# lightalchemist/nonlocal-image-edit

Hardware: AMD Instinct MI355X
Metric: megapixels/sec end-to-end enhance (4K img, m=200, K=50); device-resident input and output (host->host per SURVEY 8d: host_to_host.value) (higher is better)
Workload: dtype f64; 1 GPU; cfg4: 4096x4096 synthetic luminance, 20x10 samples (p=200), K=50, T=10, L=4 layers; device-resident: the luminance plane is in HBM when the timed region starts and the 4 layer planes are left in HBM (no PCIe inside `value`); parallelism=single GPU, formulation=phi_free_tables, storage=fp64 tables, histograms, reductions and MFMA; fp32 output planes

## Files before the change

### include/nle.h

```cpp
#ifndef NLE_H
#define NLE_H

#include <stddef.h>

#ifdef __cplusplus
extern "C" {
#endif

#define NLE_OK 0
#define NLE_ERR_INVALID 1
#define NLE_ERR_HIP 2
#define NLE_ERR_NUMERIC 3
#define NLE_ERR_COMM 4

#define NLE_EPS 1e-10

typedef struct nle_ctx nle_ctx;
typedef struct nle_filter nle_filter;

int nle_ctx_create(int device, void* stream, nle_ctx** out);
void nle_ctx_destroy(nle_ctx* ctx);
const char* nle_last_error(const nle_ctx* ctx);
int nle_ctx_synchronize(nle_ctx* ctx);
int nle_ctx_trim(nle_ctx* ctx);
// ... 87 lines not shown
                         double hy, int form, double thresh, float* d_r, double* h_summary);
int nle_ts_gemm64(nle_ctx* ctx, const double* d_A, long long M, int lda, int kd, const double* h_B, int nc, double* d_C);
int nle_sinkhorn_scalings64(nle_ctx* ctx, const double* d_phi, long long M, int ld, int r, const double* h_eigvals,
                            int max_iter, double* h_u_c, double* h_u_r);
int nle_gram64(nle_ctx* ctx, const double* d_phi, long long M, int ld, int r, const double* h_u, double* h_G);
int nle_row_scalings64(nle_ctx* ctx, const double* d_phi, long long M, int ld, int r, const double* h_u, double* d_out);
int nle_sample_pass(nle_ctx* ctx, const float* d_lum, int H, int W, int n_row_samples, int n_col_samples, double hx, double hy,
                    int row0, int row1, int recip, const double* h_w, double* d_y, double* h_z);
int nle_sample_gram(nle_ctx* ctx, const float* d_lum, int H, int W, int n_row_samples, int n_col_samples, double hx, double hy,
                    int row0, int row1, const double* d_c, double* h_G);
int nle_sample_project(nle_ctx* ctx, const float* d_lum, int H, int W, int n_row_samples, int n_col_samples, double hx,
                       double hy, int row0, int row1, const double* h_D, int K, const double* d_c, float* d_V, int ldv);
int nle_sample_update(nle_ctx* ctx, int p, int r, int chol, int recip, const double* h_X1, const double* h_X2,
                      const double* h_lam, const double* h_z, int zrows, int zld, const double* h_sA, double* h_v, double* h_u,
                      double* h_sA_next, double* h_w_next);
long long nle_table_workspace(int n_sel_rows, int n_sel_cols, int nrows, int gram);
int nle_table_levels(nle_ctx* ctx, const float* d_x, long long n, int* h_bad, unsigned* h_mask);
int nle_table_build(nle_ctx* ctx, const float* d_lum, int H, int W, int n_row_samples, int n_col_samples, int row0, int row1,
                    double hx, double hy, const double* d_er, const double* d_ecT, const double* d_Ep, const double* d_cvec,
                    double* d_er_out, double* d_ecT_out, double* d_Ep_out, int* h_info);
int nle_table_pass(nle_ctx* ctx, const float* d_lum, int H, int W, int n_row_samples, int n_col_samples, int row0, int row1,
                   double hx, double hy, const double* d_er, const double* d_ecT, const double* d_Ep, const double* d_cvec,
                   int mode, const double* d_w, const float* d_xvec, double* d_y, double* d_ws, long long ws_elems, double* d_z);
int nle_table_expand(nle_ctx* ctx, const float* d_lum, int H, int W, int n_row_samples, int n_col_samples, int row0, int row1,
                     double hx, double hy, const double* d_er, const double* d_ecT, const double* d_Ep, const double* d_cvec,
                     const double* d_wl, int ldw, int nl, int round8, double* d_gws, float* d_out, long long ostride);
int nle_table_gram(nle_ctx* ctx, const float* d_lum, int H, int W, int n_row_samples, int n_col_samples, int row0, int row1,
                   double hx, double hy, const double* d_er, const double* d_ecT, const double* d_Ep, const double* d_cvec,
                   double* d_ws, long long ws_elems, double* d_Gk, int* h_split);
int nle_table_apply_small(nle_ctx* ctx, int p, int K, int ldk, int L, int ldw, const double* d_m, const double* d_D,
// ... 132 lines not shown
```

### nonlocal-image-edit_amd/__init__.py

```python
from __future__ import annotations

import ctypes as C
import os

import numpy as np

_HERE = os.path.dirname(os.path.abspath(__file__))
LIB_PATH = os.path.join(_HERE, "lib", "libnle_hip.so")

from . import _abi
from ._abi import (ALLREDUCE_FN, NLE_ERR_COMM, NLE_ERR_HIP, NLE_ERR_INVALID, NLE_ERR_NUMERIC, NLE_OK)

EPS = 1e-10
KERNEL_COUNT = _abi.NLE_KERNEL_COUNT
_P = C.c_void_p
_SIGNATURES = _abi.SIGNATURES
EXPORTED_SYMBOLS = tuple(_SIGNATURES)
MODE_AUTO, MODE_MATERIALISED, MODE_PHI_FREE, MODE_PHI_FREE_EXP, MODE_MATERIALISED_F64, MODE_STREAMED_F64 = (
    _abi.NLE_MODE_AUTO, _abi.NLE_MODE_MATERIALISED, _abi.NLE_MODE_PHI_FREE, _abi.NLE_MODE_PHI_FREE_EXP,
    _abi.NLE_MODE_MATERIALISED_F64, _abi.NLE_MODE_STREAMED_F64)
MODE_EXACT_F64 = _abi.NLE_MODE_EXACT_F64
EXACT_MAX_PIXELS = _abi.NLE_EXACT_MAX_PIXELS
SAMPLER_GRID, SAMPLER_FARTHEST = _abi.NLE_SAMPLER_GRID, _abi.NLE_SAMPLER_FARTHEST
SAMPLER_RESIDUAL = _abi.NLE_SAMPLER_RESIDUAL
# ... 638 lines not shown
        X1c, X2r = np.asfortranarray(X), np.ascontiguousarray(np.asarray(X2, dtype=np.float64))
        n2, r = X.shape
        p = n2 // 2
        lam = np.ascontiguousarray(lam, dtype=np.float64)
        z = np.ascontiguousarray(np.atleast_2d(z), dtype=np.float64)
        sA = None if sA is None else np.ascontiguousarray(sA, dtype=np.float64)
        if n2 != 2 * p or X2r.shape != (n2, r) or lam.size != r or z.shape[1] < p or (sA is not None and sA.size != p):
            raise NLEError(NLE_ERR_INVALID, "sample_update: X1, X2 (2p x r), lam (r), z (zrows x zld >= p), sA (p)")
        v, u, sn, wn = np.zeros(n2), np.zeros(r), np.zeros(p), np.zeros(p)
        self._sync_in()
        _check(lib().nle_sample_update(self._h, p, r, int(bool(chol)), int(sA is not None), _np_ptr(X1c), _np_ptr(X2r),
                                       _np_ptr(lam), _np_ptr(z), z.shape[0], z.shape[1], _np_ptr(sA) if sA is not None else None,
                                       _np_ptr(v), _np_ptr(u), _np_ptr(sn), _np_ptr(wn)), self._h)
        return v, u, sn, wn

    def _dev64(self, a, what, n=None):
        if a is None:
            return None
        torch = _torch()
        t = torch.as_tensor(a, dtype=torch.float64, device=f"cuda:{self.device}").contiguous()
        if n is not None and t.numel() != n:
            raise NLEError(NLE_ERR_INVALID, f"{what}: need {n} doubles, got {t.numel()}")
        return t

    def _table_view(self, lum, nr, nc, rows, tables, hx, hy, c, who):
        t, H, W = self._plane(lum)
        row0, row1 = rows if rows is not None else (0, H)
        g = sample_grid(H, W, nr, nc)
        nR, nC, nrows = g["n_sel_rows"], g["n_sel_cols"], max(row1 - row0, 0)
        keep = [t]
# ... 606 lines not shown
```

### nonlocal-image-edit_amd/_abi.py

```python
import ctypes as C

_P = C.c_void_p

NLE_OK = 0
NLE_ERR_INVALID = 1
NLE_ERR_HIP = 2
NLE_ERR_NUMERIC = 3
NLE_ERR_COMM = 4
NLE_MODE_AUTO = 0
NLE_MODE_MATERIALISED = 1
NLE_MODE_PHI_FREE = 2
NLE_MODE_PHI_FREE_EXP = 3
NLE_MODE_MATERIALISED_F64 = 4
NLE_MODE_STREAMED_F64 = 5
NLE_MODE_EXACT_F64 = 6
NLE_EXACT_MAX_PIXELS = 1048576
NLE_PATCH_RADIUS_MAX = 7
NLE_CHROMA_PATCH_RADIUS_MAX = 3
NLE_SAMPLER_GRID = 0
NLE_SAMPLER_FARTHEST = 1
NLE_SAMPLER_RESIDUAL = 3
NLE_RCCL_UNIQUE_ID_BYTES = 128
NLE_RESID_AUTO = 0
NLE_RESID_ROWS = 1
# ... 73 lines not shown
    "nle_nystrom": (C.c_int, [_P, _P, C.c_int, C.c_int, C.c_int, C.c_int, C.c_double, C.c_double, _P, _P, _P]),
    "nle_ts_gemm": (C.c_int, [_P, _P, C.c_longlong, C.c_int, C.c_int, _P, C.c_int, _P]),
    "nle_sinkhorn_scalings": (C.c_int, [_P, _P, C.c_longlong, C.c_int, C.c_int, _P, C.c_int, _P, _P]),
    "nle_gram": (C.c_int, [_P, _P, C.c_longlong, C.c_int, C.c_int, _P, _P]),
    "nle_row_scalings": (C.c_int, [_P, _P, C.c_longlong, C.c_int, C.c_int, _P, _P]),
    "nle_compute_kernel64": (C.c_int, [_P, _P, C.c_int, C.c_int, C.c_int, C.c_int, C.c_double, C.c_double, _P, _P]),
    "nle_nystrom_residual": (C.c_int, [_P, _P, C.c_int, C.c_int, C.c_int, C.c_int, C.c_double, C.c_double, C.c_int, C.c_double, _P, _P]),
    "nle_ts_gemm64": (C.c_int, [_P, _P, C.c_longlong, C.c_int, C.c_int, _P, C.c_int, _P]),
    "nle_sinkhorn_scalings64": (C.c_int, [_P, _P, C.c_longlong, C.c_int, C.c_int, _P, C.c_int, _P, _P]),
    "nle_gram64": (C.c_int, [_P, _P, C.c_longlong, C.c_int, C.c_int, _P, _P]),
    "nle_row_scalings64": (C.c_int, [_P, _P, C.c_longlong, C.c_int, C.c_int, _P, _P]),
    "nle_sample_pass": (C.c_int, [_P, _P, C.c_int, C.c_int, C.c_int, C.c_int, C.c_double, C.c_double, C.c_int, C.c_int, C.c_int, _P, _P, _P]),
    "nle_sample_gram": (C.c_int, [_P, _P, C.c_int, C.c_int, C.c_int, C.c_int, C.c_double, C.c_double, C.c_int, C.c_int, _P, _P]),
    "nle_sample_project": (C.c_int, [_P, _P, C.c_int, C.c_int, C.c_int, C.c_int, C.c_double, C.c_double, C.c_int, C.c_int, _P, C.c_int, _P, _P, C.c_int]),
    "nle_sample_update": (C.c_int, [_P, C.c_int, C.c_int, C.c_int, C.c_int, _P, _P, _P, _P, C.c_int, C.c_int, _P, _P, _P, _P, _P]),
    "nle_table_workspace": (C.c_longlong, [C.c_int, C.c_int, C.c_int, C.c_int]),
    "nle_table_levels": (C.c_int, [_P, _P, C.c_longlong, _P, _P]),
    "nle_table_build": (C.c_int, [_P, _P, C.c_int, C.c_int, C.c_int, C.c_int, C.c_int, C.c_int, C.c_double, C.c_double, _P, _P, _P, _P, _P, _P, _P, _P]),
    "nle_table_pass": (C.c_int, [_P, _P, C.c_int, C.c_int, C.c_int, C.c_int, C.c_int, C.c_int, C.c_double, C.c_double, _P, _P, _P, _P, C.c_int, _P, _P, _P, _P, C.c_longlong, _P]),
    "nle_table_expand": (C.c_int, [_P, _P, C.c_int, C.c_int, C.c_int, C.c_int, C.c_int, C.c_int, C.c_double, C.c_double, _P, _P, _P, _P, _P, C.c_int, C.c_int, C.c_int, _P, _P, C.c_longlong]),
    "nle_table_gram": (C.c_int, [_P, _P, C.c_int, C.c_int, C.c_int, C.c_int, C.c_int, C.c_int, C.c_double, C.c_double, _P, _P, _P, _P, _P, C.c_longlong, _P, _P]),
    "nle_table_apply_small": (C.c_int, [_P, C.c_int, C.c_int, C.c_int, C.c_int, C.c_int, _P, _P, _P, _P, _P, _P, _P, _P, _P, _P, _P]),
    "nle_table_scatter": (C.c_int, [_P, C.c_int, C.c_int, _P, _P, _P, C.c_longlong, C.c_int]),
    "nle_gemm64s": (C.c_int, [_P, C.c_int, C.c_int, C.c_int, _P, C.c_longlong, C.c_longlong, _P, C.c_longlong, C.c_longlong, _P, C.c_longlong, C.c_longlong, _P, _P, _P, _P, C.c_longlong, C.c_longlong]),
    "nle_gemm64s_window": (C.c_int, []),
    "nle_affinity_product64": (C.c_int, [_P, _P, C.c_int, C.c_int, C.c_double, C.c_double, _P, C.c_int, C.c_int, _P]),
    "nle_train": (C.c_int, [_P, _P, C.c_int, C.c_int, C.c_int, C.c_int, C.c_double, C.c_double, C.c_int, C.c_int, _P]),
    "nle_train_host": (C.c_int, [_P, _P, C.c_int, C.c_int, C.c_int, C.c_int, C.c_double, C.c_double, C.c_int, C.c_int, _P]),
    "nle_train_host_u8": (C.c_int, [_P, _P, C.c_int, C.c_int, C.c_int, C.c_int, C.c_double, C.c_double, C.c_int, C.c_int, _P]),
    "nle_filter_destroy": (None, [_P]),
# ... 49 lines not shown
```

### nonlocal-image-edit_amd/csrc/fused.hip

```cpp
#include "kernels.h"
#include "launch.h"

#include <algorithm>

namespace nlek {

typedef float f32x16 __attribute__((ext_vector_type(16)));

template <int MASK>
__device__ __forceinline__ void fold_level(float& a, float& b, int lane) {
    if constexpr (MASK == 32) {
        auto r = __builtin_amdgcn_permlane32_swap(__float_as_uint(a), __float_as_uint(b), false, false);
        a = __uint_as_float(r[0]) + __uint_as_float(r[1]);
    } else if constexpr (MASK == 16) {
        auto r = __builtin_amdgcn_permlane16_swap(__float_as_uint(a), __float_as_uint(b), false, false);
        a = __uint_as_float(r[0]) + __uint_as_float(r[1]);
    } else {
        const bool hi = (lane & MASK) != 0;
        const float keep = hi ? b : a, give = hi ? a : b;
        a = keep + __shfl_xor(give, MASK);
    }
}

template <int N, int LEN, int W>
// ... 162 lines not shown
    if (lane == 0) {
        if (o < p) w_next[o] = chol ? sum + v[p + o] : sum;
        else sA_next[o - p] = chol ? v[o - p] + sum : sum;
    }
}

hipError_t sink_update(hipStream_t s, int mode, int p, int r, bool chol, const double* d_X1, const double* d_X2,
                       const double* d_lam, const double* d_z, int zrows, int zld, const double* d_sA_cur, double eps,
                       double* d_v, double* d_u, double* d_sA_next, double* d_w_next) {
    const size_t shm = (size_t)2 * p * sizeof(double);
    hipLaunchKernelGGL(k_sink_update_a, dim3((unsigned)((r + 3) / 4)), dim3(256), shm, s, mode, p, r, d_X1, d_lam, d_z,
                       zrows, zld, d_sA_cur, eps, d_v, d_u);
    hipLaunchKernelGGL(k_sink_update_b, dim3((unsigned)((2 * p + 3) / 4)), dim3(256), 0, s, p, r, chol ? 1 : 0, d_X2, d_u,
                       d_v, d_sA_next, d_w_next);
    return hipGetLastError();
}

typedef double f64x4 __attribute__((ext_vector_type(4)));
constexpr int kG64Rows = 32;

int gram64_ld(int p) { return (p + 15) & ~15; }
int gram64_num_tiles(int p) {
    const int nt = gram64_ld(p) / 16;
    return nt * (nt + 1) / 2;
}
static int gram64_chunk_rows(long long M) {
    long long fl = (M + 511) / 512;
    fl = ((fl + kG64Rows - 1) / kG64Rows) * kG64Rows;
    return (int)std::max<long long>(fl, kG64Rows);
}
// ... 372 lines not shown
```

### nonlocal-image-edit_amd/csrc/handoff.h

```cpp
#pragma once
#include <hip/hip_runtime.h>

namespace nlek {
namespace handoff {

typedef unsigned long long u64;
constexpr u64 kUnset = ~0ull;
constexpr unsigned kSpinLimit = 1u << 22;

__device__ __forceinline__ u64 ld_pub(const double* p) {
    return __hip_atomic_load(reinterpret_cast<const u64*>(p), __ATOMIC_RELAXED, __HIP_MEMORY_SCOPE_AGENT);
}
__device__ __forceinline__ void st_pub(double* p, double v) {
    __hip_atomic_store(reinterpret_cast<u64*>(p), (u64)__double_as_longlong(v), __ATOMIC_RELAXED, __HIP_MEMORY_SCOPE_AGENT);
}
__device__ __forceinline__ double wait_pub(const double* p, const int* status, bool& fail) {
    u64 b;
    unsigned spins = 0;
    while ((b = ld_pub(p)) == kUnset) {
        if (++spins > kSpinLimit) {
            fail = true;
            break;
        }
        if ((spins & 1023u) == 0 &&
            __hip_atomic_load(status, __ATOMIC_RELAXED, __HIP_MEMORY_SCOPE_AGENT) != 0) {
            fail = true;
            break;
        }
        __builtin_amdgcn_s_sleep(1);
    }
    return __longlong_as_double((long long)b);
}

}
}
```

### nonlocal-image-edit_amd/csrc/kernels.h

```cpp
#pragma once
#include <hip/hip_runtime.h>

#include <vector>

namespace nlek {

struct GridSpec {
    int H, W;
    int rowStep, rowOff, nSelRows;
    int colStep, colOff, nSelCols;
    __host__ __device__ int p() const { return nSelRows * nSelCols; }
};

typedef float4 Sample4;

#if defined(__HIPCC__)
__device__ __forceinline__ float affinity_value(float pr, float pc, float px, Sample4 s, float nsw, float npw) {
    const float dr = pr - s.x, dc = pc - s.y, dv = px - s.z;
    return __builtin_amdgcn_exp2f(nsw * (dr * dr + dc * dc) + npw * (dv * dv));
}
__device__ __forceinline__ double recip_or_zero_d(double s, double eps) {
    return (fabs(s) >= eps) ? 1.0 / s : 0.0;
}
__device__ __forceinline__ bool is_sample_pixel(const GridSpec& gs, int row, int col) {
// ... 54 lines not shown
int gram_chunk_rows(long long M);
size_t gram_partial_elems(long long M, int ld);
hipError_t gram(hipStream_t s, const float* d_X, long long M, int ld, const double* d_u,
                double eps, double* d_partial, double* d_tiles);
hipError_t gram_reduce(hipStream_t s, const double* d_partial, int nchunks, int ntiles, double* d_tiles);

int sink_pass_ld(int p);
int sink_pass_rows(long long M);
int sink_pass_max_p();
hipError_t sink_pass(hipStream_t s, int mode, const float* d_lum, GridSpec gs, const Sample4* d_samples,
                     int p, const double* d_w, float nsw, float npw, long long pix0, long long M, double eps,
                     double* d_ybuf, double* d_partial);
hipError_t sink_update(hipStream_t s, int mode, int p, int r, bool chol, const double* d_X1, const double* d_X2,
                       const double* d_lam, const double* d_z, int zrows, int zld, const double* d_sA_cur, double eps,
                       double* d_v, double* d_u, double* d_sA_next, double* d_w_next);
constexpr int kG64TilesPerWave = 23;
int gram64_ld(int p);
int gram64_num_tiles(int p);
size_t gram64_partial_elems(long long M, int p);
hipError_t gram64(hipStream_t s, const float* d_lum, GridSpec gs, const Sample4* d_samples, int p, float nsw,
                  float npw, long long pix0, long long M, const double* d_c, double* d_partial, double* d_tiles);
int project64_ld(int K);
hipError_t project64(hipStream_t s, const float* d_lum, GridSpec gs, const Sample4* d_samples, int p, float nsw,
                     float npw, long long pix0, long long M, const double* d_D, int K, const double* d_c, float* d_V,
                     int ldv);

inline bool tables_apply(GridSpec gs, int K = 1) {
    return gs.nSelRows >= 1 && gs.nSelRows <= 32 && gs.nSelCols >= 1 && gs.nSelCols <= 36 && K <= 128;
}
hipError_t check_levels(hipStream_t s, const float* d_lum, long long n, int* d_flag);
// ... 129 lines not shown
hipError_t sorted_pass(hipStream_t s, int mode, GridSpec gs, int row0, int nrows, const SortedRows& sr, const double* d_g,
                       double eps, double* d_ybuf, double* d_h, const double* d_cvec, const float* d_xvec,
                       const int* d_run_if = nullptr);
bool sorted_moments_ok(GridSpec gs, double hx);
constexpr int kPlanesPerLaunch = 4;
struct PlaneGroup {
    const float* x[kPlanesPerLaunch];
    double* h[kPlanesPerLaunch];
};
int sorted_planes_per_launch(GridSpec gs);
hipError_t sorted_reduce_planes(hipStream_t s, GridSpec gs, int row0, int nrows, const SortedRows& sr, const double* d_cvec,
                                const PlaneGroup& pg, int np);
hipError_t sorted_gram_rows(hipStream_t s, GridSpec gs, int nrows, const SortedRows& sr, const double* d_cvec, double* d_Aout);

size_t hist_tiled_workspace_elems(GridSpec gs, int nrows_local);
hipError_t sink_hist_tiled(hipStream_t s, int mode, const TableView& v, const double* d_w, double eps, double* d_ybuf,
                           double* d_ws, double* d_z, LaunchObserver* obs = nullptr, const float* d_xvec = nullptr,
                           const int* d_run_if = nullptr);
size_t apply_reduce_planes_workspace_elems(GridSpec gs, int nrows_local, int np);
hipError_t apply_reduce_planes(hipStream_t s, const TableView& v, const float* const* d_x, int np, double* d_ws, double* d_m,
                               LaunchObserver* obs = nullptr);
int apply_layers_per_launch(const TableView& v);
hipError_t apply_hist_layers(hipStream_t s, const TableView& v, const double* d_wl, int ldw, int nl, double* d_ws, float* d_out,
                             long long ostride, LaunchObserver* obs, bool round8 = false);
hipError_t apply_small(hipStream_t s, int p, int K, int ldk, int L, int ldw, const double* d_m, const double* d_D,
                       const double* d_Vrows, const double* d_xA , const double* d_resp,
                       double* d_t, double* d_Wp, double* d_YA, const int* d_differs = nullptr, const double* d_m_same = nullptr,
                       const double* d_xA_same = nullptr);
hipError_t scatter_samples(hipStream_t s, int p, int L, const long long* d_loc, const double* d_YA, float* d_Y,
                           long long ystride, bool round8 = false);

size_t ghist_workspace_elems(GridSpec gs, int nrows_local);
hipError_t gram_hist(hipStream_t s, const TableView& v, double* d_ws, double* d_Gk, LaunchObserver* obs = nullptr);
// ... 69 lines not shown
```

### nonlocal-image-edit_amd/csrc/literal.hip

```cpp
#include "train.h"

using namespace nlep;

namespace {
std::vector<float> build_B(const Nystrom& n, int p) {
    std::vector<float> B((size_t)p * n.ldr, 0.f);
    for (int k = 0; k < n.r; ++k) {
        const double inv = recip0(n.lam[k]);
        for (int s = 0; s < p; ++s) B[(size_t)s * n.ldr + k] = (float)(n.VA[(size_t)k * p + s] * inv);
    }
    return B;
}

void build_phi(nle_ctx* c, const float* d_lum, const SampleSet& ss, const Nystrom& ny, double hx,
               double hy, long long pix0, long long M, float* d_phi) {
    const int p = ss.p;
    DevBuf<float4> d_samples = upload_samples(c, ss);
    std::vector<float> B = build_B(ny, p);
    DevBuf<float> d_B(B.size());
    HIP_OK(hipMemcpyAsync(d_B.p, B.data(), B.size() * sizeof(float), hipMemcpyHostToDevice, c->stream));
    const float sw = nsw_of(hx), pw = nsw_of(hy);
    if (c->nystrom_bf16x3 || c->sw.nystrom_bf16x3) {
        DevBuf<unsigned short> d_Bs(nlek::ts_gemm_bf16x3_bsplit_elems(p, ny.ldr));
        HIP_OK(nlek::ts_gemm_bf16x3_split(c->stream, d_B.p, p, ny.ldr, d_Bs.p));
// ... 617 lines not shown
        DevBuf<double> d_X1 = uploaded(ctx, h_X1, n2 * r), d_X2 = uploaded(ctx, h_X2, n2 * r), d_lam = uploaded(ctx, h_lam, (size_t)r),
                       d_z = uploaded(ctx, h_z, (size_t)zrows * zld), d_sA, d_uv(n2 + r), d_out(n2);
        if (recip) d_sA = uploaded(ctx, h_sA, (size_t)p);
        PROFILED(ctx, NLE_K_SMALL,
                 nlek::sink_update(ctx->stream, recip ? nlek::ROWPASS_RECIP : nlek::ROWPASS_COLSUM, p, r, chol != 0, d_X1.p, d_X2.p,
                                   d_lam.p, d_z.p, zrows, zld, d_sA.p, NLE_EPS, d_uv.p, d_uv.p + n2, d_out.p, d_out.p + p));
        HIP_OK(hipMemcpyAsync(h_v, d_uv.p, n2 * sizeof(double), hipMemcpyDeviceToHost, ctx->stream));
        HIP_OK(hipMemcpyAsync(h_u, d_uv.p + n2, r * sizeof(double), hipMemcpyDeviceToHost, ctx->stream));
        HIP_OK(hipMemcpyAsync(h_sA_next, d_out.p, p * sizeof(double), hipMemcpyDeviceToHost, ctx->stream));
        HIP_OK(hipMemcpyAsync(h_w_next, d_out.p + p, p * sizeof(double), hipMemcpyDeviceToHost, ctx->stream));
        HIP_OK(hipStreamSynchronize(ctx->stream));
        prof_flush(ctx);
    });
}

#define NLE_TABLE_PARAMS                                                                                                    \
    nle_ctx *ctx, const float *d_lum, int H, int W, int n_row_samples, int n_col_samples, int row0, int row1, double hx,   \
        double hy, const double *d_er, const double *d_ecT, const double *d_Ep, const double *d_cvec
#define NLE_TABLE_ARGS TableArgs{d_lum, H, W, n_row_samples, n_col_samples, row0, row1, hx, hy, d_er, d_ecT, d_Ep, d_cvec}

long long nle_table_workspace(int n_sel_rows, int n_sel_cols, int nrows, int gram) {
    if (n_sel_rows < 1 || n_sel_rows > 32 || n_sel_cols < 1 || n_sel_cols > 36 || nrows < 1) return -1;
    GridSpec gs{};
    gs.nSelRows = n_sel_rows, gs.nSelCols = n_sel_cols;
    return (long long)(gram ? nlek::ghist_workspace_elems(gs, nrows) : nlek::hist_tiled_workspace_elems(gs, nrows));
}

int nle_table_levels(nle_ctx* ctx, const float* d_x, long long n, int* h_bad, unsigned* h_mask) {
    if (!ctx || !d_x || n < 1 || !h_bad || !h_mask) return NLE_ERR_INVALID;
    return guard(ctx, [&] {
// ... 172 lines not shown
```

### nonlocal-image-edit_amd/csrc/sample_space.hip

```cpp
#include "train.h"

using namespace nlep;

namespace {
void build_update_operands(nle_ctx* c, const Nystrom& ny, int p, DevBuf<double>& d_X1, DevBuf<double>& d_X2,
                           DevBuf<double>& d_lam) {
    const int r = ny.r;
    if (ny.dev) {
        const size_t n2 = (size_t)2 * p, pp = (size_t)p * p;
        d_X1.alloc(n2 * p);
        d_X2.alloc(n2 * p);
        d_lam.alloc(p);
        HIP_OK(hipMemsetAsync(d_X1.p, 0, n2 * p * sizeof(double), c->stream));
        HIP_OK(nlek::transpose64(c->stream, p, ny.dev->ch.Linv.p, d_X1.p, p, 2 * p));
        HIP_OK(hipMemcpyAsync(d_X2.p, ny.dev->ch.Linv.p, pp * sizeof(double), hipMemcpyDeviceToDevice, c->stream));
        HIP_OK(hipMemcpyAsync(d_X2.p + pp, ny.dev->Ka.p, pp * sizeof(double), hipMemcpyDeviceToDevice, c->stream));
        HIP_OK(nlek::fill64(c->stream, d_lam.p, p, 1.0));
    } else {
        const size_t n2 = (size_t)2 * p;
        std::vector<double> X1(n2 * r, 0.0), X2(n2 * r);
        for (int k = 0; k < r; ++k)
            for (int a = 0; a < p; ++a) {
                const double b = ny.B[(size_t)k * p + a];
                const double va = ny.chol ? ny.Ka[(size_t)k * p + a] : ny.VA[(size_t)k * p + a];
// ... 3 lines not shown
                X2[(size_t)(p + a) * r + k] = va;
            }
        d_X1.alloc(X1.size());
        d_X2.alloc(X2.size());
        d_lam.alloc(r);
        HIP_OK(hipMemcpyAsync(d_X1.p, X1.data(), X1.size() * sizeof(double), hipMemcpyHostToDevice, c->stream));
        HIP_OK(hipMemcpyAsync(d_X2.p, X2.data(), X2.size() * sizeof(double), hipMemcpyHostToDevice, c->stream));
        HIP_OK(hipMemcpyAsync(d_lam.p, ny.lam.data(), r * sizeof(double), hipMemcpyHostToDevice, c->stream));
        HIP_OK(hipStreamSynchronize(c->stream));
    }
}

struct SampleSinkhorn {
    nle_ctx* c;
    int p, T, zld;
    DevBuf<double> d_w, d_sAh, d_X1, d_X2, d_lam, d_uv;
    std::vector<double> sA_c, sA_r;

    SampleSinkhorn(nle_ctx* c_, int p_, int zld_, int T_)
        : c(c_), p(p_), T(T_), zld(zld_), d_w(zld_), d_sAh((size_t)2 * T_ * p_), d_uv((size_t)3 * p_) {
        HIP_OK(hipMemsetAsync(d_w.p, 0, zld * sizeof(double), c->stream));
    }

    Nystrom run(const SolveKa& solve, const std::function<void(int, bool)>& pass_pixels, double* d_z, int zrows) {
        pass_pixels(nlek::ROWPASS_COLSUM, false);
        Nystrom ny = solve();
        build_update_operands(c, ny, p, d_X1, d_X2, d_lam);
        auto update = [&](int n, int mode) {
            all_reduce(c, d_z, (size_t)zrows * zld);
            PROFILED(c, NLE_K_SMALL,
                     nlek::sink_update(c->stream, mode, p, ny.r, ny.chol, d_X1.p, d_X2.p, d_lam.p, d_z, zrows, zld,
                                       n > 0 ? d_sAh.p + (size_t)(n - 1) * p : nullptr, NLE_EPS, d_uv.p, d_uv.p + 2 * p,
                                       d_sAh.p + (size_t)n * p, d_w.p));
        };
        update(0, nlek::ROWPASS_COLSUM);
        for (int n = 1; n < 2 * T; ++n) {
            pass_pixels(nlek::ROWPASS_RECIP, n == 2 * T - 1);
            update(n, nlek::ROWPASS_RECIP);
        }
        sA_c.resize(p);
        sA_r.resize(p);
        HIP_OK(hipMemcpyAsync(sA_c.data(), d_sAh.p + (size_t)(2 * T - 2) * p, p * sizeof(double), hipMemcpyDeviceToHost,
                              c->stream));
        HIP_OK(hipMemcpyAsync(sA_r.data(), d_sAh.p + (size_t)(2 * T - 1) * p, p * sizeof(double), hipMemcpyDeviceToHost,
                              c->stream));
        return ny;
    }
};

OrthoSS ortho_ss_host(nle_ctx* c, const Nystrom& ny, int p, const SampleSinkhorn& sk, const std::function<void()>& enqueue_gram,
                      double* d_G, size_t g_elems, bool tile16, int n_eig, Timer& tm_g, double* host_ms, Trace& tr) {
    OrthoSS o;
    enqueue_gram();
    ortho_ss_prepare(o, ny, p, sk.sA_c, sk.sA_r, c->topk_solver != 0, c->sw.force_eig, tr.on);
    tr.mark("ss: ortho prepare (host)");
    all_reduce(c, d_G, g_elems);
    std::vector<double> tiles(g_elems);
    HIP_OK(hipMemcpyAsync(tiles.data(), d_G, tiles.size() * sizeof(double), hipMemcpyDeviceToHost, c->stream));
    tm_g.stop();
// ... 63 lines not shown
    if (lum || !sorted_rows() || nrows <= 0) return lum;
    dst.alloc((size_t)nrows * gs.W);
    PROFILED(ctx, NLE_K_SMALL, nlek::rows_from_sorted(ctx->stream, gs, row0, nrows, sorted, samples.p, p, dst.p));
    return dst.p - (long long)row0 * gs.W;
}
void nlep::TableFilter::ensure_plane(nle_ctx* ctx) { lum = plane_into(ctx, slab); }

namespace nlep {

void TrainPath::train_tables(const SolveKa& solve) {
    const int p = ss.p;
    tm_s.start();
    auto t = std::make_unique<TableFilter>(c, d_lum, ss, hx, hy, (int)(pix0 / ss.gs.W), (int)(M / ss.gs.W));
    const nlek::TableView view = t->view();
    DevBuf<double> d_z(t->P64), d_hws(nlek::hist_tiled_workspace_elems(ss.gs, t->nrows));
    SampleSinkhorn sk(c, p, t->P64, T);
    tr.mark("ss: alloc+upload");
    auto pass_pixels = [&](int mode, bool last) {
        ProfObserver obs(c, kProfTablePass);
        HIP_OK(nlek::sink_hist_tiled(c->stream, mode, view, sk.d_w.p, NLE_EPS, last ? t->c.p : nullptr, d_hws.p, d_z.p, &obs));
    };
    const Nystrom ny = sk.run(solve, pass_pixels, d_z.p, 1);
    adopt_nystrom(f, ny, NLE_MODE_PHI_FREE);
    tm_s.stop();
    tr.mark("ss: passes enqueued");
    HIP_OK(hipStreamSynchronize(c->stream));
    tr.mark("ss: sinkhorn sync");

    tm_g.start();
    const size_t g_elems = (size_t)p * p;
    DevBuf<double> d_gpart, d_G(g_elems);
    auto enqueue_gram = [&] {
        d_gpart.alloc(nlek::ghist_workspace_elems(ss.gs, t->nrows));
        {
            ProfObserver obs(c, kProfTableGram);
            HIP_OK(nlek::gram_hist(c->stream, view, d_gpart.p, d_G.p, &obs));
        }
        if (t->lev.p) {
            t->m_train.alloc(t->P64);
            t->xA_train.alloc(p);
            {
                ProfObserver obs(c, kProfTableReduce);
// ... 331 lines not shown
```

### nonlocal-image-edit_amd/csrc/tables.hip

```cpp
#include "kernels.h"
#include "launch.h"

#include <algorithm>

namespace nlek {

typedef double f64x4 __attribute__((ext_vector_type(4)));

constexpr int kLevels = 256;

constexpr int kGroupMin = 12;
constexpr int kGroupRounds = 3;

template <int CTRL, int ROW_MASK>
__device__ __forceinline__ double dpp_f64(double v) {
    int lo = __double2loint(v), hi = __double2hiint(v);
    lo = __builtin_amdgcn_update_dpp(0, lo, CTRL, ROW_MASK, 0xf, true);
    hi = __builtin_amdgcn_update_dpp(0, hi, CTRL, ROW_MASK, 0xf, true);
    return __hiloint2double(hi, lo);
}
__device__ __forceinline__ double wave_sum63(double v) {
    v += dpp_f64<0xB1, 0xf>(v);
    v += dpp_f64<0x4E, 0xf>(v);
    v += dpp_f64<0x141, 0xf>(v);
// ... 420 lines not shown
    const int want = std::max(1, (4096 + ncoltiles - 1) / ncoltiles);
    int rows = (nrows_local + want - 1) / want;
    rows = std::max(64, ((rows + 31) / 32) * 32);
    const int lds_rows = ((8192 / std::max(gs.nSelRows, 1)) / 32) * 32;
    return std::min(rows, std::max(64, lds_rows));
}
size_t hist_tiled_workspace_elems(GridSpec gs, int nrows_local) {
    const size_t n = (size_t)kLevels * gs.nSelCols;
    const int sr = hist_slab_rows(gs, nrows_local);
    const int nslabs = (nrows_local + sr - 1) / sr;
    const size_t ldp = ((size_t)gs.nSelRows * gs.nSelCols + 63) & ~(size_t)63;
    return 2 * (size_t)nrows_local * n + (size_t)nslabs * std::max(n * gs.nSelRows, (size_t)(kLevels / 16) * ldp);
}

static hipError_t launch_hist_hh_z(hipStream_t s, const TableView& v, const double* d_h, double* d_HH, double* d_z,
                                   const int* d_run_if = nullptr) {
    const GridSpec gs = v.gs;
    const int nC = gs.nSelCols, nR = gs.nSelRows, p = v.p, ldp = v.ldp, nrows_local = v.nrows;
    const int slab_rows = hist_slab_rows(gs, nrows_local), nslabs = (nrows_local + slab_rows - 1) / slab_rows;
    const int lev_t0 = v.sorted ? v.sorted->lev_t0 : 0, lev_nt = v.sorted ? v.sorted->lev_nt : kLevels / 16;
    const size_t shm_hh = (size_t)slab_rows * nR * sizeof(double);
    hipError_t e = launch(k_hist_hh, dim3((unsigned)((nC * lev_nt + 3) / 4), (unsigned)nslabs), dim3(256), shm_hh, s, nC, nR,
                          nrows_local, slab_rows, lev_t0, lev_nt, v.er, d_h, v.Ep, p, ldp, d_HH, d_run_if);
    if (e != hipSuccess) return e;
    hipLaunchKernelGGL(k_z_reduce, dim3((unsigned)((ldp + 7) / 8)), dim3(256), 0, s, d_HH, nslabs * lev_nt, p, ldp, d_z, d_run_if);
    return hipGetLastError();
}

hipError_t sink_hist_tiled(hipStream_t s, int mode, const TableView& v, const double* d_w, double eps, double* d_ybuf,
                           double* d_ws, double* d_z, LaunchObserver* obs, const float* d_xvec, const int* d_run_if) {
    if (!tables_apply(v.gs) || (d_run_if != nullptr && v.sorted == nullptr)) return hipErrorInvalidValue;
    const GridSpec gs = v.gs;
    const int nC = gs.nSelCols, p = v.p, row0 = v.row0, nrows_local = v.nrows;
    const SortedRows* sorted = v.sorted;
    const double* d_cvec = mode == ROWPASS_XVEC ? v.cvec : nullptr;
    struct Scope {
        LaunchObserver* o;
        Scope(LaunchObserver* ob, int sub) : o(ob) { if (o) o->begin(sub); }
        ~Scope() { if (o) o->end(); }
    };
    const size_t n = (size_t)kLevels * nC;
    double* d_g = d_ws;
    double* d_h = d_g + (size_t)nrows_local * n;
    double* d_HH = d_h + (size_t)nrows_local * n;
    const int lev_t0 = sorted ? sorted->lev_t0 : 0, lev_nt = sorted ? sorted->lev_nt : kLevels / 16;
    if (mode == ROWPASS_RECIP) {
// ... 4 lines not shown
    if (sorted != nullptr) {
        Scope sc(obs, SUB_HIST_PIX);
        hipError_t ep = sorted_pass(s, mode, gs, row0, nrows_local, *sorted, d_g, eps, d_ybuf, d_h, d_cvec, d_xvec, d_run_if);
        if (ep != hipSuccess) return ep;
    } else {
        Scope sc(obs, SUB_HIST_PIX);
        hipError_t ep = hipErrorInvalidValue;
        dispatch_columns<1, 36>(nC, [&](auto nc) {
            constexpr int NC = decltype(nc)::value;
            ep = launch(k_hist_pix<NC>, dim3((unsigned)nrows_local), dim3(kPixThreads), (size_t)2 * kLevels * (NC | 1) * sizeof(double),
                        s, mode, v.lum, gs, row0, v.ecT, d_g, eps, d_ybuf, d_h, d_cvec, d_xvec);
        });
        if (ep != hipSuccess) return ep;
    }
    Scope sc(obs, SUB_HIST_HH);
    return launch_hist_hh_z(s, v, d_h, d_HH, d_z, d_run_if);
}

size_t apply_reduce_planes_workspace_elems(GridSpec gs, int nrows_local, int np) {
    return hist_tiled_workspace_elems(gs, nrows_local) + (size_t)std::max(np - 2, 0) * nrows_local * kLevels * gs.nSelCols;
}

hipError_t apply_reduce_planes(hipStream_t s, const TableView& v, const float* const* d_x, int np, double* d_ws, double* d_m,
                               LaunchObserver* obs) {
    if (!tables_apply(v.gs) || v.sorted == nullptr || np < 2 || np > sorted_planes_per_launch(v.gs)) return hipErrorInvalidValue;
    const size_t tab = (size_t)v.nrows * kLevels * v.gs.nSelCols;
    double* d_HH = d_ws + (size_t)np * tab;
    PlaneGroup pg{};
    for (int m = 0; m < np; ++m) pg.x[m] = d_x[m], pg.h[m] = d_ws + (size_t)m * tab;
    if (obs) obs->begin(SUB_HIST_PIX);
    hipError_t ep = sorted_reduce_planes(s, v.gs, v.row0, v.nrows, *v.sorted, v.cvec, pg, np);
// ... 442 lines not shown
```

Before: 3643 MP/s.

## Fuse Sinkhorn z-reduce and update into one cross-workgroup step kernel

```diff
diff --git a/include/nle.h b/include/nle.h
--- a/include/nle.h
+++ b/include/nle.h
@@ -125,6 +125,9 @@
 int nle_sample_update(nle_ctx* ctx, int p, int r, int chol, int recip, const double* h_X1, const double* h_X2,
                       const double* h_lam, const double* h_z, int zrows, int zld, const double* h_sA, double* h_v, double* h_u,
                       double* h_sA_next, double* h_w_next);
+int nle_sample_step(nle_ctx* ctx, int p, int r, int chol, int recip, const double* h_X1, const double* h_X2, const double* h_lam,
+                    const double* h_zpart, int nparts, int ldp, const double* h_sA, int nsteps, int rounds, double* h_z,
+                    double* h_v, double* h_u, double* h_sA_next, double* h_w_next);
 long long nle_table_workspace(int n_sel_rows, int n_sel_cols, int nrows, int gram);
 int nle_table_levels(nle_ctx* ctx, const float* d_x, long long n, int* h_bad, unsigned* h_mask);
 int nle_table_build(nle_ctx* ctx, const float* d_lum, int H, int W, int n_row_samples, int n_col_samples, int row0, int row1,
diff --git a/nonlocal-image-edit_amd/__init__.py b/nonlocal-image-edit_amd/__init__.py
--- a/nonlocal-image-edit_amd/__init__.py
+++ b/nonlocal-image-edit_amd/__init__.py
@@ -676,6 +676,26 @@
                                        _np_ptr(v), _np_ptr(u), _np_ptr(sn), _np_ptr(wn)), self._h)
         return v, u, sn, wn
 
+    def sample_step(self, X1, X2, lam, zpart, sA=None, chol=False, rounds=1):
+        X = np.asarray(X1, dtype=np.float64)
+        X1c, X2r = np.asfortranarray(X), np.ascontiguousarray(np.asarray(X2, dtype=np.float64))
+        n2, r = X.shape
+        p = n2 // 2
+        lam = np.ascontiguousarray(lam, dtype=np.float64)
+        zp = np.ascontiguousarray(zpart, dtype=np.float64)
+        squeeze = zp.ndim == 2 and rounds == 1
+        zp = zp.reshape((-1,) + zp.shape[-2:])
+        nsteps, nparts, ldp = zp.shape
+        sA = None if sA is None else np.ascontiguousarray(sA, dtype=np.float64)
+        if n2 != 2 * p or X2r.shape != (n2, r) or lam.size != r or ldp != (p + 63) & ~63 or (sA is not None and sA.size != p):
+            raise NLEError(NLE_ERR_INVALID, "sample_step: X1, X2 (2p x r), lam (r), zpart (nsteps x nparts x ldp), sA (p)")
+        out = [np.zeros((rounds, nsteps, n)) for n in (ldp, n2, r, p, p)]
+        self._sync_in()
+        _check(lib().nle_sample_step(self._h, p, r, int(bool(chol)), int(sA is not None), _np_ptr(X1c), _np_ptr(X2r), _np_ptr(lam),
+                                     _np_ptr(zp), nparts, ldp, _np_ptr(sA) if sA is not None else None, nsteps, int(rounds),
+                                     *(_np_ptr(o) for o in out)), self._h)
+        return tuple(o[0, 0] for o in out) if squeeze else tuple(out)
+
     def _dev64(self, a, what, n=None):
         if a is None:
             return None
diff --git a/nonlocal-image-edit_amd/_abi.py b/nonlocal-image-edit_amd/_abi.py
--- a/nonlocal-image-edit_amd/_abi.py
+++ b/nonlocal-image-edit_amd/_abi.py
@@ -111,6 +111,7 @@
     "nle_sample_gram": (C.c_int, [_P, _P, C.c_int, C.c_int, C.c_int, C.c_int, C.c_double, C.c_double, C.c_int, C.c_int, _P, _P]),
     "nle_sample_project": (C.c_int, [_P, _P, C.c_int, C.c_int, C.c_int, C.c_int, C.c_double, C.c_double, C.c_int, C.c_int, _P, C.c_int, _P, _P, C.c_int]),
     "nle_sample_update": (C.c_int, [_P, C.c_int, C.c_int, C.c_int, C.c_int, _P, _P, _P, _P, C.c_int, C.c_int, _P, _P, _P, _P, _P]),
+    "nle_sample_step": (C.c_int, [_P, C.c_int, C.c_int, C.c_int, C.c_int, _P, _P, _P, _P, C.c_int, C.c_int, _P, C.c_int, C.c_int, _P, _P, _P, _P, _P]),
     "nle_table_workspace": (C.c_longlong, [C.c_int, C.c_int, C.c_int, C.c_int]),
     "nle_table_levels": (C.c_int, [_P, _P, C.c_longlong, _P, _P]),
     "nle_table_build": (C.c_int, [_P, _P, C.c_int, C.c_int, C.c_int, C.c_int, C.c_int, C.c_int, C.c_double, C.c_double, _P, _P, _P, _P, _P, _P, _P, _P]),
diff --git a/nonlocal-image-edit_amd/csrc/fused.hip b/nonlocal-image-edit_amd/csrc/fused.hip
--- a/nonlocal-image-edit_amd/csrc/fused.hip
+++ b/nonlocal-image-edit_amd/csrc/fused.hip
@@ -1,3 +1,4 @@
+#include "handoff.h"
 #include "kernels.h"
 #include "launch.h"
 
@@ -200,6 +201,179 @@
     hipLaunchKernelGGL(k_sink_update_b, dim3((unsigned)((2 * p + 3) / 4)), dim3(256), 0, s, p, r, chol ? 1 : 0, d_X2, d_u,
                        d_v, d_sA_next, d_w_next);
     return hipGetLastError();
+}
+
+__global__ __launch_bounds__(256) void k_sink_step(int mode, int p, int r, int chol, int ldp, const double* __restrict__ zpart,
+                                                   int nparts, const double* __restrict__ X1, const double* __restrict__ X2,
+                                                   const double* __restrict__ lam, const double* __restrict__ sA_cur, double eps,
+                                                   double* __restrict__ z_out, double* __restrict__ v_out,
+                                                   double* __restrict__ u_out, double* __restrict__ sA_next,
+                                                   double* __restrict__ w_next, double* pub, int* status) {
+    extern __shared__ __attribute__((aligned(16))) unsigned char smem_raw[];
+    __shared__ double sm[32][8];
+    double* v = reinterpret_cast<double*>(smem_raw);
+    const int tid = threadIdx.x, lane = tid & 63, wave = tid >> 6, n2 = 2 * p, wg = blockIdx.x;
+    const int k = wg * 4 + wave;
+    const bool colsum = mode == ROWPASS_COLSUM;
+    double* pub_z = pub;
+    double* pub_u = pub + p;
+    constexpr int kStepPre = 8, kStepZ = 12;
+    const double* col = X1 + (size_t)k * n2;
+    const double* row = X2 + (size_t)k * r;
+    double c_pre[kStepPre], r_pre[kStepPre];
+#pragma unroll
+    for (int e = 0; e < kStepPre; ++e) {
+        const int i = lane + 64 * e;
+        c_pre[e] = (k < r && i < n2) ? col[i] : 0.0;
+        r_pre[e] = (k < n2 && i < r) ? row[i] : 0.0;
+    }
+    const double lam_k = (k < r && lane == 0) ? lam[k] : 0.0;
+    if (wg < (ldp + 7) / 8) {
+        const int c = tid & 7, g = tid >> 3, zc = wg * 8 + c;
+        double s = 0.0;
+        if (zc < p)
+            for (int q0 = g; q0 < nparts; q0 += 32 * kStepZ) {
+                double t[kStepZ];
+#pragma unroll
+                for (int e = 0; e < kStepZ; ++e) t[e] = zpart[(size_t)min(q0 + 32 * e, nparts - 1) * ldp + zc];
+#pragma unroll
+                for (int e = 0; e < kStepZ; ++e)
+                    if (q0 + 32 * e < nparts) s += t[e];
+            }
+        sm[g][c] = s;
+        __syncthreads();
+        if (g == 0 && zc < ldp) {
+            double t = 0.0;
+#pragma unroll
+            for (int q = 0; q < 32; ++q) t += sm[q][c];
+            z_out[zc] = t;
+            if (zc < p) handoff::st_pub(pub_z + zc, t);
+        }
+    }
+    if (wg < (r + 3) / 4) {
+        bool fail = false;
+        for (int a0 = tid; a0 < p; a0 += 4 * 256) {
+            handoff::u64 zb[4];
+            double ya[4];
+#pragma unroll
+            for (int e = 0; e < 4; ++e) zb[e] = handoff::ld_pub(pub_z + min(a0 + 256 * e, p - 1));
+#pragma unroll
+            for (int e = 0; e < 4; ++e) ya[e] = colsum ? 1.0 : sA_cur[min(a0 + 256 * e, p - 1)];
+#pragma unroll
+            for (int e = 0; e < 4; ++e) ya[e] = colsum ? 1.0 : recip_or_zero_d(ya[e], eps);
+#pragma unroll
+            for (int e = 0; e < 4; ++e) {
+                const int a = a0 + 256 * e;
+                if (a < p) {
+                    const double t = handoff::wait_pub_from(zb[e], pub_z + a, status, fail);
+                    v[a] = t;
+                    v[p + a] = ya[e];
+                    if (wg == 0) {
+                        v_out[a] = t;
+                        v_out[p + a] = ya[e];
+                    }
+                }
+            }
+        }
+        if (__syncthreads_or(fail)) {
+            if (tid == 0) __hip_atomic_store(status, 1, __ATOMIC_RELAXED, __HIP_MEMORY_SCOPE_AGENT);
+            return;
+        }
+        if (k < r) {
+            double s0 = 0.0, s1 = 0.0;
+            for (int e0 = 0; lane + 64 * e0 < n2; e0 += kStepPre) {
+                double cc[kStepPre];
+#pragma unroll
+                for (int e = 0; e < kStepPre; ++e) {
+                    const int i = lane + 64 * (e0 + e);
+                    if (i < n2) cc[e] = e0 == 0 ? c_pre[e] : col[i];
+                }
+#pragma unroll
+                for (int e = 0; e < kStepPre; ++e) {
+                    const int i = lane + 64 * (e0 + e);
+                    if (i < n2) {
+                        if (e & 1) s1 += cc[e] * v[i];
+                        else s0 += cc[e] * v[i];
+                    }
+                }
+            }
+            double sum = s0 + s1;
+#pragma unroll
+            for (int off = 32; off > 0; off >>= 1) sum += __shfl_xor(sum, off);
+            if (lane == 0) {
+                const double uk = lam_k * sum;
+                u_out[k] = uk;
+                handoff::st_pub(pub_u + k, uk);
+            }
+        }
+    }
+    const int o = k;
+    if (o >= n2) return;
+    bool fail = false;
+    const bool exact = chol != 0 && o >= p;
+    const bool add_z = chol != 0 && lane == 0 && o >= p;
+    handoff::u64 zb = 0;
+    if (add_z) zb = handoff::ld_pub(pub_z + (o - p));
+    double s0 = 0.0, s1 = 0.0;
+    for (int e0 = 0; lane + 64 * e0 < r; e0 += kStepPre) {
+        double rr[kStepPre], xx[kStepPre];
+        handoff::u64 ub[kStepPre];
+#pragma unroll
+        for (int e = 0; e < kStepPre; ++e) {
+            const int i = lane + 64 * (e0 + e);
+            const int ic = min(i, r - 1);
+            rr[e] = e0 == 0 ? r_pre[e] : row[ic];
+            if (exact) xx[e] = colsum ? 1.0 : recip_or_zero_d(sA_cur[ic], eps);
+            else ub[e] = handoff::ld_pub(pub_u + ic);
+        }
+#pragma unroll
+        for (int e = 0; e < kStepPre; ++e) {
+            const int i = lane + 64 * (e0 + e);
+            if (i < r) {
+                const double x = exact ? xx[e] : handoff::wait_pub_from(ub[e], pub_u + i, status, fail);
+                if (e & 1) s1 += rr[e] * x;
+                else s0 += rr[e] * x;
+            }
+        }
+    }
+    double sum = s0 + s1;
+#pragma unroll
+    for (int off = 32; off > 0; off >>= 1) sum += __shfl_xor(sum, off);
+    double add = 0.0;
+    if (chol != 0 && lane == 0) {
+        if (o < p) add = colsum ? 1.0 : recip_or_zero_d(sA_cur[o], eps);
+        else add = handoff::wait_pub_from(zb, pub_z + (o - p), status, fail);
+    }
+    if (__any(fail)) {
+        if (lane == 0) __hip_atomic_store(status, 1, __ATOMIC_RELAXED, __HIP_MEMORY_SCOPE_AGENT);
+        return;
+    }
+    if (lane == 0) {
+        if (o < p) w_next[o] = chol ? sum + add : sum;
+        else sA_next[o - p] = chol ? add + sum : sum;
+    }
+}
+
+static unsigned sink_step_grid(int p, int ldp) { return (unsigned)std::max((ldp + 7) / 8, (2 * p + 3) / 4); }
+static size_t sink_step_lds(int p) { return (size_t)2 * p * sizeof(double); }
+
+bool sink_step_fits(int p, int ldp) {
+    int dev = 0, cus = 0, per_cu = 0;
+    if (p < 1 || ldp < p || hipGetDevice(&dev) != hipSuccess ||
+        hipDeviceGetAttribute(&cus, hipDeviceAttributeMultiprocessorCount, dev) != hipSuccess)
+        return false;
+    const size_t shm = sink_step_lds(p);
+    if (shm > 48 * 1024) return false;
+    if (hipOccupancyMaxActiveBlocksPerMultiprocessor(&per_cu, k_sink_step, 256, shm) != hipSuccess) return false;
+    return (long long)sink_step_grid(p, ldp) <= (long long)cus * std::min(per_cu - 1, 4);
+}
+
+hipError_t sink_step(hipStream_t s, int mode, int p, int r, bool chol, int ldp, const double* d_zpart, int nparts,
+                     const double* d_X1, const double* d_X2, const double* d_lam, const double* d_sA_cur, double eps,
+                     double* d_z, double* d_v, double* d_u, double* d_sA_next, double* d_w_next, double* d_pub, int* d_status) {
+    if (r < 1 || r > 2 * p) return hipErrorInvalidValue;
+    return launch(k_sink_step, dim3(sink_step_grid(p, ldp)), dim3(256), sink_step_lds(p), s, mode, p, r, chol ? 1 : 0, ldp, d_zpart,
+                  nparts, d_X1, d_X2, d_lam, d_sA_cur, eps, d_z, d_v, d_u, d_sA_next, d_w_next, d_pub, d_status);
 }
 
 typedef double f64x4 __attribute__((ext_vector_type(4)));
diff --git a/nonlocal-image-edit_amd/csrc/handoff.h b/nonlocal-image-edit_amd/csrc/handoff.h
--- a/nonlocal-image-edit_amd/csrc/handoff.h
+++ b/nonlocal-image-edit_amd/csrc/handoff.h
@@ -31,6 +31,9 @@
     }
     return __longlong_as_double((long long)b);
 }
+__device__ __forceinline__ double wait_pub_from(u64 b, const double* p, const int* status, bool& fail) {
+    return b == kUnset ? wait_pub(p, status, fail) : __longlong_as_double((long long)b);
+}
 
 }
 }
diff --git a/nonlocal-image-edit_amd/csrc/kernels.h b/nonlocal-image-edit_amd/csrc/kernels.h
--- a/nonlocal-image-edit_amd/csrc/kernels.h
+++ b/nonlocal-image-edit_amd/csrc/kernels.h
@@ -92,6 +92,10 @@
 hipError_t sink_update(hipStream_t s, int mode, int p, int r, bool chol, const double* d_X1, const double* d_X2,
                        const double* d_lam, const double* d_z, int zrows, int zld, const double* d_sA_cur, double eps,
                        double* d_v, double* d_u, double* d_sA_next, double* d_w_next);
+bool sink_step_fits(int p, int ldp);
+hipError_t sink_step(hipStream_t s, int mode, int p, int r, bool chol, int ldp, const double* d_zpart, int nparts,
+                     const double* d_X1, const double* d_X2, const double* d_lam, const double* d_sA_cur, double eps,
+                     double* d_z, double* d_v, double* d_u, double* d_sA_next, double* d_w_next, double* d_pub, int* d_status);
 constexpr int kG64TilesPerWave = 23;
 int gram64_ld(int p);
 int gram64_num_tiles(int p);
@@ -251,9 +255,13 @@
 hipError_t sorted_gram_rows(hipStream_t s, GridSpec gs, int nrows, const SortedRows& sr, const double* d_cvec, double* d_Aout);
 
 size_t hist_tiled_workspace_elems(GridSpec gs, int nrows_local);
+struct ZPartials {
+    const double* rows;
+    int nparts;
+};
 hipError_t sink_hist_tiled(hipStream_t s, int mode, const TableView& v, const double* d_w, double eps, double* d_ybuf,
                            double* d_ws, double* d_z, LaunchObserver* obs = nullptr, const float* d_xvec = nullptr,
-                           const int* d_run_if = nullptr);
+                           const int* d_run_if = nullptr, ZPartials* zparts = nullptr);
 size_t apply_reduce_planes_workspace_elems(GridSpec gs, int nrows_local, int np);
 hipError_t apply_reduce_planes(hipStream_t s, const TableView& v, const float* const* d_x, int np, double* d_ws, double* d_m,
                                LaunchObserver* obs = nullptr);
diff --git a/nonlocal-image-edit_amd/csrc/literal.hip b/nonlocal-image-edit_amd/csrc/literal.hip
--- a/nonlocal-image-edit_amd/csrc/literal.hip
+++ b/nonlocal-image-edit_amd/csrc/literal.hip
@@ -655,6 +655,48 @@
     });
 }
 
+int nle_sample_step(nle_ctx* ctx, int p, int r, int chol, int recip, const double* h_X1, const double* h_X2, const double* h_lam,
+                    const double* h_zpart, int nparts, int ldp, const double* h_sA, int nsteps, int rounds, double* h_z,
+                    double* h_v, double* h_u, double* h_sA_next, double* h_w_next) {
+    if (!ctx || !h_X1 || !h_X2 || !h_lam || !h_zpart || !h_z || !h_v || !h_u || !h_sA_next || !h_w_next || p < 1 || r < 1 ||
+        r > p || nparts < 1 || ldp < p || ldp % 64 != 0 || nsteps < 1 || rounds < 1 || (recip && !h_sA) || (chol && r != p))
+        return NLE_ERR_INVALID;
+    return guard(ctx, [&] {
+        HIP_OK(hipSetDevice(ctx->device));
+        if (!nlek::sink_step_fits(p, ldp)) throw Fail{NLE_ERR_INVALID, "nle_sample_step: the step kernel's grid does not fit on the device at once"};
+        const size_t n2 = (size_t)2 * p, nz = (size_t)nparts * ldp, slot = (size_t)p + r;
+        DevBuf<double> d_X1 = uploaded(ctx, h_X1, n2 * r), d_X2 = uploaded(ctx, h_X2, n2 * r), d_lam = uploaded(ctx, h_lam, (size_t)r),
+                       d_zpart = uploaded(ctx, h_zpart, nsteps * nz), d_sA, d_pub(nsteps * slot), d_z((size_t)nsteps * ldp),
+                       d_v(nsteps * n2), d_u((size_t)nsteps * r), d_sAn((size_t)nsteps * p), d_wn((size_t)nsteps * p);
+        DevBuf<int> d_status(1);
+        if (recip) d_sA = uploaded(ctx, h_sA, (size_t)p);
+        int st = 0;
+        for (int round = 0; round < rounds && st == 0; ++round) {
+            HIP_OK(hipMemsetAsync(d_pub.p, 0xFF, d_pub.n * sizeof(double), ctx->stream));
+            HIP_OK(hipMemsetAsync(d_status.p, 0, sizeof(int), ctx->stream));
+            for (DevBuf<double>* o : {&d_z, &d_v, &d_u, &d_sAn, &d_wn}) fill_nan(ctx, o->p, o->n);
+            for (int n = 0; n < nsteps; ++n) {
+                const bool rc = n > 0 || recip;
+                PROFILED(ctx, NLE_K_SMALL,
+                         nlek::sink_step(ctx->stream, rc ? nlek::ROWPASS_RECIP : nlek::ROWPASS_COLSUM, p, r, chol != 0, ldp,
+                                         d_zpart.p + n * nz, nparts, d_X1.p, d_X2.p, d_lam.p, n > 0 ? d_sAn.p + (size_t)(n - 1) * p : d_sA.p,
+                                         NLE_EPS, d_z.p + (size_t)n * ldp, d_v.p + n * n2, d_u.p + (size_t)n * r, d_sAn.p + (size_t)n * p,
+                                         d_wn.p + (size_t)n * p, d_pub.p + n * slot, d_status.p));
+            }
+            const size_t k = (size_t)round * nsteps;
+            HIP_OK(hipMemcpyAsync(&st, d_status.p, sizeof(int), hipMemcpyDeviceToHost, ctx->stream));
+            HIP_OK(hipMemcpyAsync(h_z + k * ldp, d_z.p, d_z.n * sizeof(double), hipMemcpyDeviceToHost, ctx->stream));
+            HIP_OK(hipMemcpyAsync(h_v + k * n2, d_v.p, d_v.n * sizeof(double), hipMemcpyDeviceToHost, ctx->stream));
+            HIP_OK(hipMemcpyAsync(h_u + k * r, d_u.p, d_u.n * sizeof(double), hipMemcpyDeviceToHost, ctx->stream));
+            HIP_OK(hipMemcpyAsync(h_sA_next + k * p, d_sAn.p, d_sAn.n * sizeof(double), hipMemcpyDeviceToHost, ctx->stream));
+            HIP_OK(hipMemcpyAsync(h_w_next + k * p, d_wn.p, d_wn.n * sizeof(double), hipMemcpyDeviceToHost, ctx->stream));
+            HIP_OK(hipStreamSynchronize(ctx->stream));
+        }
+        prof_flush(ctx);
+        if (st != 0) throw Fail{NLE_ERR_NUMERIC, "nle_sample_step: a hand-off between the workgroups of the step kernel timed out"};
+    });
+}
+
 #define NLE_TABLE_PARAMS                                                                                                    \
     nle_ctx *ctx, const float *d_lum, int H, int W, int n_row_samples, int n_col_samples, int row0, int row1, double hx,   \
         double hy, const double *d_er, const double *d_ecT, const double *d_Ep, const double *d_cvec
diff --git a/nonlocal-image-edit_amd/csrc/sample_space.hip b/nonlocal-image-edit_amd/csrc/sample_space.hip
--- a/nonlocal-image-edit_amd/csrc/sample_space.hip
+++ b/nonlocal-image-edit_amd/csrc/sample_space.hip
@@ -41,12 +41,29 @@
 struct SampleSinkhorn {
     nle_ctx* c;
     int p, T, zld;
-    DevBuf<double> d_w, d_sAh, d_X1, d_X2, d_lam, d_uv;
+    DevBuf<double> d_w, d_X1, d_X2, d_lam, d_uv, d_pub;
+    double* d_sAh;
     std::vector<double> sA_c, sA_r;
-
-    SampleSinkhorn(nle_ctx* c_, int p_, int zld_, int T_)
-        : c(c_), p(p_), T(T_), zld(zld_), d_w(zld_), d_sAh((size_t)2 * T_ * p_), d_uv((size_t)3 * p_) {
-        HIP_OK(hipMemsetAsync(d_w.p, 0, zld * sizeof(double), c->stream));
+    bool step = false;
+    nlek::ZPartials zparts{};
+
+    SampleSinkhorn(nle_ctx* c_, int p_, int zld_, int T_, bool table_path = false)
+        : c(c_), p(p_), T(T_), zld(zld_), d_w((size_t)zld_ + (size_t)2 * T_ * p_ + 1), d_uv((size_t)3 * p_),
+          d_sAh(d_w.p + zld_) {
+        HIP_OK(hipMemsetAsync(d_w.p, 0, d_w.n * sizeof(double), c->stream));
+        step = table_path && c->world == 1 && !c->comm && nlek::sink_step_fits(p, zld);
+        if (step) {
+            d_pub.alloc((size_t)2 * T * 2 * p);
+            HIP_OK(hipMemsetAsync(d_pub.p, 0xFF, d_pub.n * sizeof(double), c->stream));
+        }
+    }
+    int* d_status() { return reinterpret_cast<int*>(d_sAh + (size_t)2 * T * p); }
+    void check() {
+        if (!step) return;
+        int st = 0;
+        std::memcpy(&st, &sA_r[p], sizeof st);
+        sA_r.resize(p);
+        if (st != 0) throw Fail{NLE_ERR_NUMERIC, "Sinkhorn update: a hand-off between the workgroups of the step kernel timed out"};
     }
 
     Nystrom run(const SolveKa& solve, const std::function<void(int, bool)>& pass_pixels, double* d_z, int zrows) {
@@ -54,11 +71,18 @@
         Nystrom ny = solve();
         build_update_operands(c, ny, p, d_X1, d_X2, d_lam);
         auto update = [&](int n, int mode) {
+            const double* sA_cur = n > 0 ? d_sAh + (size_t)(n - 1) * p : nullptr;
+            if (step) {
+                PROFILED(c, NLE_K_SMALL,
+                         nlek::sink_step(c->stream, mode, p, ny.r, ny.chol, zld, zparts.rows, zparts.nparts, d_X1.p, d_X2.p, d_lam.p,
+                                         sA_cur, NLE_EPS, d_z, d_uv.p, d_uv.p + 2 * p, d_sAh + (size_t)n * p, d_w.p,
+                                         d_pub.p + (size_t)n * 2 * p, d_status()));
+                return;
+            }
             all_reduce(c, d_z, (size_t)zrows * zld);
             PROFILED(c, NLE_K_SMALL,
                      nlek::sink_update(c->stream, mode, p, ny.r, ny.chol, d_X1.p, d_X2.p, d_lam.p, d_z, zrows, zld,
-                                       n > 0 ? d_sAh.p + (size_t)(n - 1) * p : nullptr, NLE_EPS, d_uv.p, d_uv.p + 2 * p,
-                                       d_sAh.p + (size_t)n * p, d_w.p));
+                                       sA_cur, NLE_EPS, d_uv.p, d_uv.p + 2 * p, d_sAh + (size_t)n * p, d_w.p));
         };
         update(0, nlek::ROWPASS_COLSUM);
         for (int n = 1; n < 2 * T; ++n) {
@@ -66,10 +90,10 @@
             update(n, nlek::ROWPASS_RECIP);
         }
         sA_c.resize(p);
-        sA_r.resize(p);
-        HIP_OK(hipMemcpyAsync(sA_c.data(), d_sAh.p + (size_t)(2 * T - 2) * p, p * sizeof(double), hipMemcpyDeviceToHost,
+        sA_r.resize(p + (step ? 1 : 0));
+        HIP_OK(hipMemcpyAsync(sA_c.data(), d_sAh + (size_t)(2 * T - 2) * p, p * sizeof(double), hipMemcpyDeviceToHost,
                               c->stream));
-        HIP_OK(hipMemcpyAsync(sA_r.data(), d_sAh.p + (size_t)(2 * T - 1) * p, p * sizeof(double), hipMemcpyDeviceToHost,
+        HIP_OK(hipMemcpyAsync(sA_r.data(), d_sAh + (size_t)(2 * T - 1) * p, sA_r.size() * sizeof(double), hipMemcpyDeviceToHost,
                               c->stream));
         return ny;
     }
@@ -163,11 +187,12 @@
     auto t = std::make_unique<TableFilter>(c, d_lum, ss, hx, hy, (int)(pix0 / ss.gs.W), (int)(M / ss.gs.W));
     const nlek::TableView view = t->view();
     DevBuf<double> d_z(t->P64), d_hws(nlek::hist_tiled_workspace_elems(ss.gs, t->nrows));
-    SampleSinkhorn sk(c, p, t->P64, T);
+    SampleSinkhorn sk(c, p, t->P64, T, true);
     tr.mark("ss: alloc+upload");
     auto pass_pixels = [&](int mode, bool last) {
         ProfObserver obs(c, kProfTablePass);
-        HIP_OK(nlek::sink_hist_tiled(c->stream, mode, view, sk.d_w.p, NLE_EPS, last ? t->c.p : nullptr, d_hws.p, d_z.p, &obs));
+        HIP_OK(nlek::sink_hist_tiled(c->stream, mode, view, sk.d_w.p, NLE_EPS, last ? t->c.p : nullptr, d_hws.p, d_z.p, &obs,
+                                     nullptr, nullptr, sk.step ? &sk.zparts : nullptr));
     };
     const Nystrom ny = sk.run(solve, pass_pixels, d_z.p, 1);
     adopt_nystrom(f, ny, NLE_MODE_PHI_FREE);
@@ -175,6 +200,7 @@
     tr.mark("ss: passes enqueued");
     HIP_OK(hipStreamSynchronize(c->stream));
     tr.mark("ss: sinkhorn sync");
+    sk.check();
 
     tm_g.start();
     const size_t g_elems = (size_t)p * p;
diff --git a/nonlocal-image-edit_amd/csrc/tables.hip b/nonlocal-image-edit_amd/csrc/tables.hip
--- a/nonlocal-image-edit_amd/csrc/tables.hip
+++ b/nonlocal-image-edit_amd/csrc/tables.hip
@@ -458,7 +458,7 @@
 }
 
 static hipError_t launch_hist_hh_z(hipStream_t s, const TableView& v, const double* d_h, double* d_HH, double* d_z,
-                                   const int* d_run_if = nullptr) {
+                                   const int* d_run_if = nullptr, ZPartials* zparts = nullptr) {
     const GridSpec gs = v.gs;
     const int nC = gs.nSelCols, nR = gs.nSelRows, p = v.p, ldp = v.ldp, nrows_local = v.nrows;
     const int slab_rows = hist_slab_rows(gs, nrows_local), nslabs = (nrows_local + slab_rows - 1) / slab_rows;
@@ -467,13 +467,18 @@
     hipError_t e = launch(k_hist_hh, dim3((unsigned)((nC * lev_nt + 3) / 4), (unsigned)nslabs), dim3(256), shm_hh, s, nC, nR,
                           nrows_local, slab_rows, lev_t0, lev_nt, v.er, d_h, v.Ep, p, ldp, d_HH, d_run_if);
     if (e != hipSuccess) return e;
+    if (zparts != nullptr) {
+        *zparts = ZPartials{d_HH, nslabs * lev_nt};
+        return hipSuccess;
+    }
     hipLaunchKernelGGL(k_z_reduce, dim3((unsigned)((ldp + 7) / 8)), dim3(256), 0, s, d_HH, nslabs * lev_nt, p, ldp, d_z, d_run_if);
     return hipGetLastError();
 }
 
 hipError_t sink_hist_tiled(hipStream_t s, int mode, const TableView& v, const double* d_w, double eps, double* d_ybuf,
-                           double* d_ws, double* d_z, LaunchObserver* obs, const float* d_xvec, const int* d_run_if) {
-    if (!tables_apply(v.gs) || (d_run_if != nullptr && v.sorted == nullptr)) return hipErrorInvalidValue;
+                           double* d_ws, double* d_z, LaunchObserver* obs, const float* d_xvec, const int* d_run_if,
+                           ZPartials* zparts) {
+    if (!tables_apply(v.gs) || (d_run_if != nullptr && (v.sorted == nullptr || zparts != nullptr))) return hipErrorInvalidValue;
     const GridSpec gs = v.gs;
     const int nC = gs.nSelCols, p = v.p, row0 = v.row0, nrows_local = v.nrows;
     const SortedRows* sorted = v.sorted;
@@ -508,7 +513,7 @@
         if (ep != hipSuccess) return ep;
     }
     Scope sc(obs, SUB_HIST_HH);
-    return launch_hist_hh_z(s, v, d_h, d_HH, d_z, d_run_if);
+    return launch_hist_hh_z(s, v, d_h, d_HH, d_z, d_run_if, zparts);
 }
 
 size_t apply_reduce_planes_workspace_elems(GridSpec gs, int nrows_local, int np) {
```

New measurement: 3574 MP/s. 0.981x the previous value.
